# pzou01/unitree-rl-gym

Measured on AMD Instinct MI355X. Metric: env-steps/sec + PPO-iter wall-time, Go2 4096 envs/GPU at 1/2/4/8 MI355X, higher is better.
Workload: dtype fp32 env step; bf16 MFMA policy GEMMs (fp32 accumulate); 1 GPU; Go2 flat terrain, 4096 envs/GPU, MLP actor-critic 512-256-128, PPO 24 steps x 5 epochs x 4 mini-batches; num_envs_per_gpu=4096, decimation=4, parallelism=dp1

## Files before the change

### unitree-rl-gym_amd/csrc/ppo_mlp.hip

```cpp
#include <hip/hip_runtime.h>

#include <algorithm>
#include <cstdint>
#include <cstdlib>
#include <type_traits>
#include <string>

#include "../../include/ppo_mlp.h"
#include "pmlp_noise.h"

typedef __bf16 bf16;
typedef bf16 bf16x8 __attribute__((ext_vector_type(8)));
typedef bf16 bf16x4 __attribute__((ext_vector_type(4)));
typedef short shortx4 __attribute__((ext_vector_type(4)));
typedef short shortx8 __attribute__((ext_vector_type(8)));
typedef __attribute__((address_space(3))) shortx4 lds_shortx4;
typedef float floatx16 __attribute__((ext_vector_type(16)));

static thread_local std::string g_err;
static int fail(int code, const std::string& m) {
    g_err = m;
    return code;
}
#define PMLP_CHECK_LAUNCH(what)                                                                       \
// ... 1463 lines not shown
#pragma unroll 8
    for (int i = threadIdx.x; i < nparts; i += PMLP_OPT_THREADS) s += partial[i];
    return block_sum(s, sh);
}
__device__ __forceinline__ size_t frag_index(int r, int c, int ld) {
    return ((((size_t)(r >> 5) * (ld >> 4) + (c >> 4)) * 64 + (r & 31) + 32 * ((c >> 3) & 1)) << 3) + (c & 7);
}
__global__ __launch_bounds__(PMLP_OPT_THREADS) void k_adam(float* __restrict__ p, const float* __restrict__ g,
                                                           float* __restrict__ m, float* __restrict__ v, int64_t n,
                                                           float scale, const float* __restrict__ partial, int nparts,
                                                           const float* step, const float* lr, float max_norm,
                                                           float b1, float b2, float eps, MirrorJobs mj) {
    __shared__ float sh[4];
    const float s = norm_partials_sum(partial, nparts, sh);
    float coef = scale;
    if (max_norm > 0.f) coef = scale * fminf(max_norm / (sqrtf(s) + 1e-6f), 1.f);
    const float t = step[0];
    const float bc1 = 1.f - powf(b1, t), bc2s = sqrtf(1.f - powf(b2, t));
    const float step_size = lr[0] / bc1;
    for (int64_t i = (int64_t)blockIdx.x * PMLP_OPT_THREADS + threadIdx.x; i < n;
         i += (int64_t)gridDim.x * PMLP_OPT_THREADS) {
        float mi = m[i], vi = v[i];
        const float pi = adam_elem(g[i], mi, vi, p[i], coef, b1, b2, eps, step_size, bc2s);
        m[i] = mi;
        v[i] = vi;
        p[i] = pi;
        for (int j = 0; j < mj.n; ++j) {
            const int64_t o = i - mj.off[j];
            if (o >= 0 && o < (int64_t)mj.rows[j] * mj.cols[j]) {
                const int oi = (int)o, r = oi / mj.cols[j], c = oi - r * mj.cols[j];
                mj.dst[j][(size_t)r * mj.ld[j] + c] = (bf16)pi;
                if (mj.frag[j]) mj.frag[j][frag_index(r, c, mj.ld[j])] = (bf16)pi;
            }
        }
    }
}

template <int VEC>
__global__ __launch_bounds__(PMLP_OPT_THREADS) void k_adam_vec(float* __restrict__ p, const float* __restrict__ g,
                                                               float* __restrict__ m, float* __restrict__ v, int64_t n,
                                                               float scale, const float* __restrict__ partial, int nparts,
                                                               const float* step, const float* lr, float max_norm,
                                                               float b1, float b2, float eps, MirrorJobs mj) {
    typedef float vf __attribute__((ext_vector_type(VEC)));
    typedef bf16 vb __attribute__((ext_vector_type(VEC)));
    __shared__ float sh[4];
    const int64_t ng = n / VEC, i0 = (int64_t)blockIdx.x * PMLP_OPT_THREADS + threadIdx.x;
    const int64_t stride = (int64_t)gridDim.x * PMLP_OPT_THREADS;
    vf G, M, V, P;
    if (i0 < ng) {
        G = ((const vf*)g)[i0];
        M = ((const vf*)m)[i0];
        V = ((const vf*)v)[i0];
        P = ((const vf*)p)[i0];
    }
    const float s = norm_partials_sum(partial, nparts, sh);
    float coef = scale;
    if (max_norm > 0.f) coef = scale * fminf(max_norm / (sqrtf(s) + 1e-6f), 1.f);
    const float t = step[0];
    const float bc1 = 1.f - powf(b1, t), bc2s = sqrtf(1.f - powf(b2, t));
    const float step_size = lr[0] / bc1;
    for (int64_t i = i0; i < ng; i += stride) {
        if (i != i0) {
            G = ((const vf*)g)[i];
            M = ((const vf*)m)[i];
            V = ((const vf*)v)[i];
            P = ((const vf*)p)[i];
        }
        vb B;
#pragma unroll
        for (int e = 0; e < VEC; ++e) {
            float me = M[e], ve = V[e];
            P[e] = adam_elem(G[e], me, ve, P[e], coef, b1, b2, eps, step_size, bc2s);
            M[e] = me;
            V[e] = ve;
            B[e] = (bf16)P[e];
        }
        ((vf*)m)[i] = M;
        ((vf*)v)[i] = V;
        ((vf*)p)[i] = P;
        const int64_t e0 = i * VEC;
        for (int j = 0; j < mj.n; ++j) {
            const int64_t o = e0 - mj.off[j];
            if (o >= 0 && o < (int64_t)mj.rows[j] * mj.cols[j]) {
                const int oi = (int)o, r = oi / mj.cols[j], c = oi - r * mj.cols[j];
                *(vb*)(mj.dst[j] + (size_t)r * mj.ld[j] + c) = B;
                if (mj.frag[j]) *(vb*)(mj.frag[j] + frag_index(r, c, mj.ld[j])) = B;
            }
        }
    }
    if (blockIdx.x == 0 && threadIdx.x < n - ng * VEC) {
        const int64_t i = ng * VEC + threadIdx.x;
        float mi = m[i], vi = v[i];
        p[i] = adam_elem(g[i], mi, vi, p[i], coef, b1, b2, eps, step_size, bc2s);
        m[i] = mi;
        v[i] = vi;
    }
}


#define FMLP_MAX_H0 512
#define FMLP_MAX_H1 256
#define FMLP_MAX_K0 256
#define FMLP_THREADS 512

struct FmlpJob {
    const float* x;
    const int64_t* rows;
    int ldx, kx;
    bf16* xa;
    int ldxa;
    const bf16* W[4];
    const float* b[4];
    int N[4];
    int K0;
    bf16* y[3];
    int ldy[3];
    float* out;
    int ldo;
    const bf16* Wf[4];
};
struct FmlpJobs {
    FmlpJob j[2];
    int njobs;
};

template <int R, bool LAST>
__device__ __forceinline__ void fmlp_layer(const bf16* A, int lda, int K, const bf16* __restrict__ W,
                                           const bf16* __restrict__ Wf,
                                           const float* __restrict__ bias, int N, bf16* D, int ldd,
                                           float* __restrict__ out, int ldo, int r0, int M) {
    constexpr int RT = R / 32, NW = FMLP_THREADS / 64;
    const int lane = threadIdx.x & 63, wid = threadIdx.x >> 6;
    const int nct = (N + 31) >> 5, ks = K >> 4;
    for (int ct = wid; ct < nct; ct += NW) {
        floatx16 acc[RT];
#pragma unroll
        for (int i = 0; i < RT; ++i)
#pragma unroll
            for (int t = 0; t < 16; ++t) acc[i][t] = 0.f;
        const int n = ct * 32 + (lane & 31);
        const bool nv = n < N;
        const bf16* wrow = Wf ? Wf + ((size_t)ct * ks * 64 + lane) * 8 : W + (size_t)(nv ? n : 0) * K + 8 * (lane >> 5);
        const int wstep = Wf ? 512 : 16;
        const bf16* arow = A + (lane & 31) * lda + 8 * (lane >> 5);
        constexpr int FG = 4;
        bf16x8 bq[FG], bn[FG];
        auto loadg = [&](int s0, bf16x8(&b)[FG]) {
#if defined(PMLP_FMLP_STAMPS) && PMLP_FMLP_STAMPS == 2
#pragma unroll
            for (int u = 0; u < FG; ++u)
#pragma unroll
                for (int e = 0; e < 8; ++e) b[u][e] = (bf16)(float)(s0 + u + e + lane);
#else
#pragma unroll
            for (int u = 0; u < FG; ++u) b[u] = *(const bf16x8*)(wrow + min(s0 + u, ks - 1) * wstep);
#endif
        };
        auto step = [&](int s, const bf16x8& b) {
#pragma unroll
            for (int i = 0; i < RT; ++i) {
                const bf16x8 af = *(const bf16x8*)(arow + i * 32 * lda + s * 16);
#if defined(PMLP_FMLP_STAMPS) && PMLP_FMLP_STAMPS == 3
                acc[i][s & 15] += (float)af[0] * (float)b[0];
#else
                acc[i] = __builtin_amdgcn_mfma_f32_32x32x16_bf16(b, af, acc[i], 0, 0, 0);
#endif
            }
        };
        auto group = [&](int s0, const bf16x8(&b)[FG]) {
#pragma unroll
            for (int u = 0; u < FG; ++u) step(s0 + u, b[u]);
        };
        auto tail = [&](int s0, const bf16x8(&b)[FG]) {
#pragma unroll
            for (int u = 0; u < FG; ++u)
                if (s0 + u < ks) step(s0 + u, b[u]);
        };
        float bq4[4][4];
#pragma unroll
        for (int q = 0; q < 4; ++q)
#pragma unroll
            for (int c = 0; c < 4; ++c)
                bq4[q][c] = bias ? bias[min(ct * 32 + 8 * q + 4 * (lane >> 5) + c, N - 1)] : 0.f;
        loadg(0, bq);
        int s0 = 0;
        for (; s0 + 2 * FG <= ks; s0 += 2 * FG) {
            loadg(s0 + FG, bn);
            group(s0, bq);
            loadg(s0 + 2 * FG, bq);
            group(s0 + FG, bn);
        }
        if (s0 < ks) {
            loadg(s0 + FG, bn);
            tail(s0, bq);
            tail(s0 + FG, bn);
        }
        const int rl = lane & 31;
#pragma unroll
        for (int q = 0; q < 4; ++q) {
            const int n0 = ct * 32 + 8 * q + 4 * (lane >> 5);
            if (LAST && n0 >= N) continue;
#pragma unroll
            for (int i = 0; i < RT; ++i) {
                const int r = i * 32 + rl;
                if constexpr (LAST) {
                    if (r0 + r < M) {
#pragma unroll
                        for (int c = 0; c < 4; ++c)
                            if (n0 + c < N) out[(size_t)(r0 + r) * ldo + n0 + c] = acc[i][4 * q + c] + bq4[q][c];
                    }
                } else {
                    bf16x4 v;
#pragma unroll
                    for (int c = 0; c < 4; ++c) v[c] = (bf16)elu(acc[i][4 * q + c] + bq4[q][c]);
                    *(bf16x4*)(D + r * ldd + n0) = v;
                }
            }
        }
    }
}

template <int R>
__device__ __forceinline__ void fmlp_store(const bf16* D, int lds_ld, int N, bf16* y, int ldy, int r0, int M) {
    if (!y) return;
    const int cpr = N >> 3;
    for (int i = threadIdx.x; i < R * cpr; i += FMLP_THREADS) {
        const int r = i / cpr, c = (i - r * cpr) * 8;
        if (r0 + r < M) *(uint4*)(y + (size_t)(r0 + r) * ldy + c) = *(const uint4*)(D + r * lds_ld + c);
    }
}

#ifdef PMLP_FMLP_STAMPS
#define FMLP_NSTAMP 20
__device__ unsigned long long g_fmlp_stamps[4096 * FMLP_NSTAMP];
#define FMLP_STAMP(k)                                                                          \
    do {                                                                                       \
        const unsigned long long t_ = __builtin_amdgcn_s_memtime();                             \
        if (threadIdx.x == 0 && blockIdx.x < 4096) g_fmlp_stamps[blockIdx.x * FMLP_NSTAMP + (k)] = t_; \
    } while (0)
extern "C" int pmlp_diag_fmlp_stamps(unsigned long long* host, int n) {
    return hipMemcpyFromSymbol(host, HIP_SYMBOL(g_fmlp_stamps), sizeof(unsigned long long) * n) == hipSuccess ? 0 : -1;
}
#else
#define FMLP_STAMP(k) ((void)(k))
#endif

struct RollStep {
    const float* stdv;
    const float* obs;
    const float* cobs;
    int O, CO, A;
    float *actions_out, *st_actions, *st_logp, *st_mu, *st_sigma, *st_value, *st_obs, *st_cobs;
    int64_t* draw;
    int parity;
    uint64_t seed;
    const float* rew;
    const uint8_t* dones;
    const uint8_t* time_outs;
    const float* prev_value;
    float* st_rew;
    uint8_t* st_dones;
    float gamma;
    pmlp_env_extras ex;
};

__device__ __forceinline__ bool ex_any(const pmlp_env_extras& x) { return x.acc[x.nsum] > 0.f; }
__device__ __forceinline__ bool ex_row(const pmlp_env_extras& x, bool any, int i, const uint8_t* time_outs) {
    bool to = false;
    if (x.carry && any) {
        const uint8_t b = x.time_out[i];
        x.carry[i] = b;
        to = b != 0;
    } else if (time_outs) {
        to = time_outs[i] != 0;
    }
    if (x.push && x.last_root_vel && !x.pushed[x.pushed[2] & 1u]) {
        x.last_root_vel[6 * (size_t)i] = x.vsim[2 * (size_t)i];
        x.last_root_vel[6 * (size_t)i + 1] = x.vsim[2 * (size_t)i + 1];
    }
    return to;
}
__device__ __forceinline__ void ex_once(const pmlp_env_extras& x, bool any, int t) {
#pragma clang fp contract(off)
    if (x.ep_means && t < x.nsum) {
        float m = x.ep_means[t];
        if (any) m = x.acc[t] / fmaxf(x.acc[x.nsum], 1.f) / x.ep_len_s;
        x.ep_means[t] = m;
        if (x.ep_snapshot) x.ep_snapshot[t] = m;
    }
    if (x.level_sum && x.ep_means && t == x.nsum) {
        float m = x.ep_means[x.nsum];
        if (any) m = (float)*x.level_sum / (float)x.num_envs;
        x.ep_means[x.nsum] = m;
        if (x.ep_snapshot) x.ep_snapshot[x.nsum] = m;
    }
    if (t <= x.nsum) x.acc_next[t] = 0.f;
    if (t == 0) {
        x.pushed[(x.pushed[2] + 1u) & 1u] = 0u;
        if (x.step_counter) *x.step_counter += 1;
    }
}

template <int R>
__device__ void roll_epilogue(const FmlpJob& J, int jj, const RollStep& rs, int r0, int M, float* terms) {
#pragma clang fp contract(off)
    const int tid = threadIdx.x;
    if (jj == 0) {
        const uint32_t draw = (uint32_t)rs.draw[rs.parity];
        const uint2 key = make_uint2((uint32_t)rs.seed, (uint32_t)(rs.seed >> 32));
        for (int q = tid; q < R * 4; q += FMLP_THREADS) {
            const int rl = q >> 2, c = q & 3, k0 = 4 * c, i = r0 + rl;
            if (i >= M || k0 >= rs.A) continue;
            const uint4 r = philox4x32(make_uint4(draw, (uint32_t)i, (uint32_t)c, 0x5050u), key);
            const float rad0 = sqrtf(-2.f * logf(u01(r.x))), rad1 = sqrtf(-2.f * logf(u01(r.z)));
            float z[4];
            sincospif(2.f * u01(r.y), &z[1], &z[0]);
            sincospif(2.f * u01(r.w), &z[3], &z[2]);
            z[0] *= rad0; z[1] *= rad0; z[2] *= rad1; z[3] *= rad1;
#pragma unroll
            for (int u = 0; u < 4; ++u) {
                const int k = k0 + u;
                if (k >= rs.A) break;
                const size_t o = (size_t)i * rs.A + k;
                const float sg = rs.stdv[k], mu = J.out[(size_t)i * J.ldo + k];
                const float act = mu + sg * z[u];
                const float d = act - mu;
                terms[rl * 16 + k] = -(d * d) / (2.f * sg * sg) - logf(sg) - kHalfLog2Pi;
                rs.actions_out[o] = act;
                rs.st_actions[o] = act;
                rs.st_mu[o] = mu;
                rs.st_sigma[o] = sg;
            }
        }
        __syncthreads();
        const bool ex = rs.rew && rs.ex.acc;
        const bool any = ex && ex_any(rs.ex);
        if (tid < R && r0 + tid < M) {
            const int i = r0 + tid;
            float logp = 0.f;
            for (int k = 0; k < rs.A; ++k) logp += terms[tid * 16 + k];
            rs.st_logp[i] = logp;
            if (rs.rew) {
                const bool to = ex ? ex_row(rs.ex, any, i, rs.time_outs) : (rs.time_outs && rs.time_outs[i]);
                float rw = rs.rew[i];
                if (rs.time_outs) rw = rw + rs.gamma * (rs.prev_value[i] * (to ? 1.f : 0.f));
                rs.st_rew[i] = rw;
                rs.st_dones[i] = rs.dones[i] ? 1 : 0;
            }
        }
        if (ex && blockIdx.x == 0) ex_once(rs.ex, any, tid);
        const int nrow = min(R, M - r0);
        for (int q = tid; q < nrow * rs.O; q += FMLP_THREADS)
            rs.st_obs[(size_t)r0 * rs.O + q] = rs.obs[(size_t)r0 * rs.O + q];
        if (blockIdx.x == 0 && tid == 0) rs.draw[rs.parity ^ 1] = (int64_t)draw + 1;
    } else {
        if (tid < R && r0 + tid < M) rs.st_value[r0 + tid] = J.out[(size_t)(r0 + tid) * J.ldo];
        if (rs.st_cobs) {
            const int nrow = min(R, M - r0);
            for (int q = tid; q < nrow * rs.CO; q += FMLP_THREADS)
                rs.st_cobs[(size_t)r0 * rs.CO + q] = rs.cobs[(size_t)r0 * rs.CO + q];
        }
    }
}

template <int R, bool ROLL = false, bool LOSS = false, bool WIDE = false>
__global__ __launch_bounds__(FMLP_THREADS) void k_mlp_fwd(FmlpJobs jobs, int M, RollStep rs, LossArgs la = {},
                                                         LossStepOut lo = {}) {
    constexpr int LD0 = FMLP_MAX_H0 + 8, LD1 = FMLP_MAX_H1 + 8;
    constexpr bool XR = R >= 96 && !WIDE;
    constexpr int LDX = 68;
    __shared__ __attribute__((aligned(16))) bf16 Y0[R * LD0];
    __shared__ __attribute__((aligned(16))) bf16 Y1[R * LD1];
    __shared__ __attribute__((aligned(16))) bf16 X[XR ? R * LDX : 8];
    bf16* const xs = XR ? X : Y1;
    const int ldxs = XR ? LDX : LD1;
    const int r0 = blockIdx.x * R;
    const int jb = gridDim.y > 1 ? blockIdx.y : 0, je = gridDim.y > 1 ? blockIdx.y + 1 : jobs.njobs;
    for (int jj = jb; jj < je; ++jj) {
        const FmlpJob& J = jobs.j[jj];
        const int sb = 9 * (jj - jb);
        FMLP_STAMP(sb + 0);
        const FmlpJob& P = jobs.j[jj > 0 ? jj - 1 : 0];
        const bool same_rows = XR && jj > jb && !J.xa && J.x == P.x && J.rows == P.rows && J.ldx == P.ldx &&
                               J.kx == P.kx && J.K0 == P.K0;
        const int cpr = J.K0 >> 3;
        for (int i = threadIdx.x; i < (same_rows ? 0 : R * cpr); i += FMLP_THREADS) {
            const int r = i / cpr, k = (i - r * cpr) * 8, m = r0 + r;
            bf16x8 t;
#pragma unroll
            for (int u = 0; u < 8; ++u) t[u] = (bf16)0.f;
            if (m < M) {
                const float* src = J.x + (size_t)(J.rows ? J.rows[m] : (int64_t)m) * J.ldx + k;
                if (k + 8 <= J.kx && (J.ldx & 3) == 0) {
                    const float4 x0 = *(const float4*)src, x1 = *(const float4*)(src + 4);
                    t[0] = (bf16)x0.x; t[1] = (bf16)x0.y; t[2] = (bf16)x0.z; t[3] = (bf16)x0.w;
                    t[4] = (bf16)x1.x; t[5] = (bf16)x1.y; t[6] = (bf16)x1.z; t[7] = (bf16)x1.w;
                } else {
#pragma unroll
                    for (int u = 0; u < 8; ++u) t[u] = k + u < J.kx ? (bf16)src[u] : (bf16)0.f;
                }
                if (J.xa) *(bf16x8*)(J.xa + (size_t)m * J.ldxa + k) = t;
            }
            *(bf16x8*)(xs + r * ldxs + k) = t;
        }
        __syncthreads();
        FMLP_STAMP(sb + 1);
        fmlp_layer<R, false>(xs, ldxs, J.K0, J.W[0], J.Wf[0], J.b[0], J.N[0], Y0, LD0, nullptr, 0, r0, M);
        FMLP_STAMP(sb + 2);
        __syncthreads();
        fmlp_store<R>(Y0, LD0, J.N[0], J.y[0], J.ldy[0], r0, M);
        FMLP_STAMP(sb + 3);
        fmlp_layer<R, false>(Y0, LD0, J.N[0], J.W[1], J.Wf[1], J.b[1], J.N[1], Y1, LD1, nullptr, 0, r0, M);
        FMLP_STAMP(sb + 4);
        __syncthreads();
        fmlp_store<R>(Y1, LD1, J.N[1], J.y[1], J.ldy[1], r0, M);
        FMLP_STAMP(sb + 5);
        fmlp_layer<R, false>(Y1, LD1, J.N[1], J.W[2], J.Wf[2], J.b[2], J.N[2], Y0, LD0, nullptr, 0, r0, M);
        FMLP_STAMP(sb + 6);
        __syncthreads();
        fmlp_store<R>(Y0, LD0, J.N[2], J.y[2], J.ldy[2], r0, M);
        FMLP_STAMP(sb + 7);
        fmlp_layer<R, true>(Y0, LD0, J.N[2], J.W[3], J.Wf[3], J.b[3], J.N[3], nullptr, 0, J.out, J.ldo, r0, M);
        __syncthreads();
        FMLP_STAMP(sb + 8);
        if constexpr (ROLL) roll_epilogue<R>(J, jj, rs, r0, M, (float*)Y1);
    }
    if constexpr (LOSS) loss_quad_rows<R / 16>(la, lo, r0, blockIdx.x, (float*)Y1);
}

__global__ __launch_bounds__(PMLP_OPT_THREADS) void k_gae(const float* __restrict__ rew,
                                                          const uint8_t* __restrict__ dones,
                                                          const float* __restrict__ values,
                                                          const float* __restrict__ last_values,
                                                          float* __restrict__ ret, float* __restrict__ adv, int T,
                                                          int N, float gamma, float lam, double* __restrict__ partial) {
#pragma clang fp contract(off)
    __shared__ double shd[2][4];
    const int e = blockIdx.x * PMLP_OPT_THREADS + threadIdx.x;
    double s1 = 0.0, s2 = 0.0;
    if (e < N) {
        float a = 0.f;
        for (int t = T - 1; t >= 0; --t) {
            const size_t i = (size_t)t * N + e;
            const float next = t == T - 1 ? last_values[e] : values[i + N];
            const float nt = 1.f - (dones[i] ? 1.f : 0.f);
            const float delta = (rew[i] + (nt * gamma) * next) - values[i];
            a = delta + ((nt * gamma) * lam) * a;
            const float r = a + values[i];
            ret[i] = r;
            const float ad = r - values[i];
            adv[i] = ad;
            s1 += ad;
            s2 += (double)ad * ad;
        }
    }
#pragma unroll
    for (int off = 32; off > 0; off >>= 1) {
        s1 += __shfl_xor(s1, off);
        s2 += __shfl_xor(s2, off);
    }
    if ((threadIdx.x & 63) == 0) {
        shd[0][threadIdx.x >> 6] = s1;
        shd[1][threadIdx.x >> 6] = s2;
    }
    __syncthreads();
    if (threadIdx.x == 0) {
        partial[2 * blockIdx.x] = (shd[0][0] + shd[0][1]) + (shd[0][2] + shd[0][3]);
        partial[2 * blockIdx.x + 1] = (shd[1][0] + shd[1][1]) + (shd[1][2] + shd[1][3]);
    }
}

__global__ __launch_bounds__(PMLP_OPT_THREADS) void k_adv_norm(float* __restrict__ adv, int64_t n,
                                                               const double* __restrict__ partial, int nparts,
                                                               const double* __restrict__ gstats) {
    __shared__ double sh[3];
    if (threadIdx.x == 0) {
        double a = 0.0, b = 0.0, c = (double)n;
        if (gstats) {
            a = gstats[0]; b = gstats[1]; c = gstats[2];
        } else {
            for (int i = 0; i < nparts; ++i) {
                a += partial[2 * i];
                b += partial[2 * i + 1];
            }
        }
        sh[0] = a;
        sh[1] = b;
        sh[2] = c;
    }
    __syncthreads();
    const double cnt = sh[2];
    const double mean = sh[0] / cnt;
    const double var = (sh[1] - cnt * mean * mean) / (cnt - 1.0);
    const float meanf = (float)mean, den = (float)sqrt(var > 0.0 ? var : 0.0) + 1e-8f;
    for (int64_t i = (int64_t)blockIdx.x * PMLP_OPT_THREADS + threadIdx.x; i < n;
         i += (int64_t)gridDim.x * PMLP_OPT_THREADS)
        adv[i] = (adv[i] - meanf) / den;
}


struct ActArgs {
    const float *mu, *stdv, *value, *obs, *cobs;
    float *actions_out, *st_actions, *st_logp, *st_mu, *st_sigma, *st_value, *st_obs, *st_cobs;
    const int64_t* draw;
    uint64_t seed;
    int N, A, O, CO;
};

__global__ __launch_bounds__(256) void k_act(ActArgs a) {
    const int64_t tid = (int64_t)blockIdx.x * blockDim.x + threadIdx.x, nth = (int64_t)gridDim.x * blockDim.x;
    const uint32_t draw = (uint32_t)*a.draw;
    const uint2 key = make_uint2((uint32_t)a.seed, (uint32_t)(a.seed >> 32));
    for (int64_t i = tid; i < a.N; i += nth) {
        float logp = 0.f;
        for (int k0 = 0; k0 < a.A; k0 += 4) {
            const uint4 r = philox4x32(make_uint4(draw, (uint32_t)i, (uint32_t)(k0 >> 2), 0x5050u), key);
            const float rad0 = sqrtf(-2.f * logf(u01(r.x))), rad1 = sqrtf(-2.f * logf(u01(r.z)));
            float z[4];
            sincospif(2.f * u01(r.y), &z[1], &z[0]);
            sincospif(2.f * u01(r.w), &z[3], &z[2]);
            z[0] *= rad0; z[1] *= rad0; z[2] *= rad1; z[3] *= rad1;
#pragma unroll
            for (int u = 0; u < 4; ++u) {
                const int k = k0 + u;
                if (k >= a.A) break;
                const size_t o = (size_t)i * a.A + k;
                const float sg = a.stdv[k], mu = a.mu[o];
                const float act = mu + sg * z[u];
                const float d = act - mu;
                logp += -(d * d) / (2.f * sg * sg) - logf(sg) - kHalfLog2Pi;
                a.actions_out[o] = act;
                a.st_actions[o] = act;
                a.st_mu[o] = mu;
                a.st_sigma[o] = sg;
            }
        }
        a.st_logp[i] = logp;
        a.st_value[i] = a.value[i];
    }
    const int64_t no = (int64_t)a.N * a.O;
    if ((no & 3) == 0 && (((uintptr_t)a.obs | (uintptr_t)a.st_obs) & 15) == 0) {
        for (int64_t j = tid; j < no / 4; j += nth) ((float4*)a.st_obs)[j] = ((const float4*)a.obs)[j];
    } else {
        for (int64_t j = tid; j < no; j += nth) a.st_obs[j] = a.obs[j];
    }
    if (a.st_cobs) {
        const int64_t nc = (int64_t)a.N * a.CO;
        for (int64_t j = tid; j < nc; j += nth) a.st_cobs[j] = a.cobs[j];
    }
}

__global__ __launch_bounds__(256) void k_act4(ActArgs a) {
    __shared__ float terms[64][16];
    const int64_t nth = (int64_t)gridDim.x * blockDim.x;
    const uint32_t draw = (uint32_t)*a.draw;
    const uint2 key = make_uint2((uint32_t)a.seed, (uint32_t)(a.seed >> 32));
    const int le = threadIdx.x >> 2, c = threadIdx.x & 3, k0 = 4 * c;
    const bool vec = (a.A & 3) == 0 &&
                     ((((uintptr_t)a.mu | (uintptr_t)a.actions_out | (uintptr_t)a.st_actions | (uintptr_t)a.st_mu |
                        (uintptr_t)a.st_sigma) & 15) == 0);
    for (int64_t base = (int64_t)blockIdx.x * blockDim.x; base < (int64_t)a.N * 4; base += nth) {
        const int64_t i = (base + threadIdx.x) >> 2;
        if (i < a.N && k0 < a.A) {
            const size_t o = (size_t)i * a.A + k0;
            float act[4], mu[4], sg[4], tm[4];
#pragma unroll
            for (int u = 0; u < 4; ++u) mu[u] = k0 + u < a.A ? a.mu[o + u] : 0.f;
            act_quad(draw, key, (uint32_t)i, c, a.A, a.stdv, mu, act, sg, tm);
#pragma unroll
            for (int u = 0; u < 4; ++u)
                if (k0 + u < a.A) terms[le][k0 + u] = tm[u];
            if (vec) {
                const float4 av = make_float4(act[0], act[1], act[2], act[3]);
                *(float4*)(a.actions_out + o) = av;
                *(float4*)(a.st_actions + o) = av;
                *(float4*)(a.st_mu + o) = make_float4(mu[0], mu[1], mu[2], mu[3]);
                *(float4*)(a.st_sigma + o) = make_float4(sg[0], sg[1], sg[2], sg[3]);
            } else {
                for (int u = 0; u < 4 && k0 + u < a.A; ++u) {
                    a.actions_out[o + u] = act[u];
                    a.st_actions[o + u] = act[u];
                    a.st_mu[o + u] = mu[u];
                    a.st_sigma[o + u] = sg[u];
                }
            }
        }
        __syncthreads();
        if (c == 0 && i < a.N) {
            float logp = 0.f;
            for (int k = 0; k < a.A; ++k) logp += terms[le][k];
            a.st_logp[i] = logp;
            a.st_value[i] = a.value[i];
        }
        __syncthreads();
    }
    const int64_t tid = (int64_t)blockIdx.x * blockDim.x + threadIdx.x;
    const int64_t no = (int64_t)a.N * a.O;
    if ((no & 3) == 0 && (((uintptr_t)a.obs | (uintptr_t)a.st_obs) & 15) == 0) {
        for (int64_t j = tid; j < no / 4; j += nth) ((float4*)a.st_obs)[j] = ((const float4*)a.obs)[j];
    } else {
        for (int64_t j = tid; j < no; j += nth) a.st_obs[j] = a.obs[j];
    }
    if (a.st_cobs) {
        const int64_t nc = (int64_t)a.N * a.CO;
        for (int64_t j = tid; j < nc; j += nth) a.st_cobs[j] = a.cobs[j];
    }
}

struct MemReset {
    float* s[PMLP_MAX_MEM_STATES];
    int n, H;
};

__global__ __launch_bounds__(256) void k_store_step(const float* __restrict__ rew, const uint8_t* __restrict__ dones,
                                                    const uint8_t* time_outs,
                                                    const float* __restrict__ st_value, float* __restrict__ st_rew,
                                                    uint8_t* __restrict__ st_dones, int N, float gamma,
                                                    int64_t* draw, MemReset mr, pmlp_env_extras ex) {
#pragma clang fp contract(off)
    const int i = blockIdx.x * blockDim.x + threadIdx.x;
    const bool any = ex.acc && ex_any(ex);
    if (ex.acc && blockIdx.x == 0) ex_once(ex, any, threadIdx.x);
    if (i < N) {
        const bool to = ex.acc ? ex_row(ex, any, i, time_outs) : (time_outs && time_outs[i]);
        float r = rew[i];
        if (time_outs) r = r + gamma * (st_value[i] * (to ? 1.f : 0.f));
        st_rew[i] = r;
        const bool d = dones[i] != 0;
        st_dones[i] = d ? 1 : 0;
        if (d)
            for (int k = 0; k < mr.n; ++k) {
                float4* h = (float4*)(mr.s[k] + (size_t)i * mr.H);
                for (int j = 0; j < mr.H / 4; ++j) h[j] = make_float4(0.f, 0.f, 0.f, 0.f);
            }
    }
    if (i == 0 && draw) *draw += 1;
}

static int g_glds = 1;
static int glds_on() {
    return g_glds;
}

template <int BM, int BN>
static bool gl_fits(int epi, int mode, const GemmBatch& gb, int njobs) {
    if (!glds_on() || (mode & 1)) return false;
    const bool tnl = epi == PMLP_EPI_PARTIAL_TN, bkn = tnl || (mode & 2);
    if (glds_on() == 2 && !tnl) return false;
    if (glds_on() == 3 && !tnl && epi != PMLP_EPI_BWD_DX) return false;
    if (epi == PMLP_EPI_PARTIAL) return false;
    if (tnl && (BM % 64 || BM > 128)) return false;
    if (bkn && (BN % 64 || BN > 128)) return false;
    for (int i = 0; i < njobs; ++i) {
        const GemmArgs& g = gb.j[i];
        if (g.K % 64 || (tnl && g.ksplit % 64)) return false;
        if (tnl && (g.M % BM || g.lda < g.M)) return false;
        if (bkn && (g.N % BN || g.ldb < g.N)) return false;
    }
    return true;
}

template <int BM, int BN, int WM, int WN>
static void launch(int epi, int mode, const GemmBatch& gb, int njobs, int maxm, int maxn, int maxk, hipStream_t st) {
    dim3 grid((maxm + BM - 1) / BM, (maxn + BN - 1) / BN, njobs * gb.slabs), block(64 * WM * WN);
    const bool af = (mode & 1) != 0, bkn = (mode & 2) != 0;
    constexpr bool km_a = BM % 64 == 0 && BM <= 128, km_b = BN % 64 == 0 && BN <= 128;
    if (gl_fits<BM, BN>(epi, mode, gb, njobs)) {
        switch (epi) {
        case PMLP_EPI_FWD_HIDDEN: hipLaunchKernelGGL((k_gemm_nt<BM, BN, WM, WN, 0, 4, 0, 1>), grid, block, 0, st, gb); return;
        case PMLP_EPI_FWD_OUT: hipLaunchKernelGGL((k_gemm_nt<BM, BN, WM, WN, 1, 4, 0, 1>), grid, block, 0, st, gb); return;
        case PMLP_EPI_BWD_DX:
            if (!bkn) {
                hipLaunchKernelGGL((k_gemm_nt<BM, BN, WM, WN, 2, 4, 0, 1>), grid, block, 0, st, gb);
                return;
            }
            if constexpr (km_b) {
                hipLaunchKernelGGL((k_gemm_nt<BM, BN, WM, WN, 2, 4, 2, 1>), grid, block, 0, st, gb);
                return;
            }
            break;
        case PMLP_EPI_PARTIAL_TN:
            if constexpr (km_a && km_b) {
                if (glds_on() >= 2) hipLaunchKernelGGL((k_gemm_nt<BM, BN, WM, WN, 4, 4, 0, 2>), grid, block, 0, st, gb);
                else hipLaunchKernelGGL((k_gemm_nt<BM, BN, WM, WN, 4, 4, 0, 1>), grid, block, 0, st, gb);
                return;
            }
            break;
        default: break;
        }
    }
    if (epi == PMLP_EPI_FWD_HIDDEN && maxk <= 48 && maxk > 32) {
        if (af) hipLaunchKernelGGL((k_gemm_nt<BM, BN, WM, WN, 0, 3, 1>), grid, block, 0, st, gb);
        else hipLaunchKernelGGL((k_gemm_nt<BM, BN, WM, WN, 0, 3>), grid, block, 0, st, gb);
        return;
    }
    if (epi == PMLP_EPI_BWD_DX && maxk <= 16) {
        if (bkn) hipLaunchKernelGGL((k_gemm_nt<BM, BN, WM, WN, 2, 1, 2>), grid, block, 0, st, gb);
        else hipLaunchKernelGGL((k_gemm_nt<BM, BN, WM, WN, 2, 1>), grid, block, 0, st, gb);
        return;
    }
    switch (epi) {
    case PMLP_EPI_FWD_HIDDEN:
        if (af) hipLaunchKernelGGL((k_gemm_nt<BM, BN, WM, WN, 0, 4, 1>), grid, block, 0, st, gb);
        else hipLaunchKernelGGL((k_gemm_nt<BM, BN, WM, WN, 0>), grid, block, 0, st, gb);
        break;
    case PMLP_EPI_FWD_OUT:
        if (af) hipLaunchKernelGGL((k_gemm_nt<BM, BN, WM, WN, 1, 4, 1>), grid, block, 0, st, gb);
        else hipLaunchKernelGGL((k_gemm_nt<BM, BN, WM, WN, 1>), grid, block, 0, st, gb);
        break;
    case PMLP_EPI_BWD_DX:
        if (bkn) hipLaunchKernelGGL((k_gemm_nt<BM, BN, WM, WN, 2, 4, 2>), grid, block, 0, st, gb);
        else hipLaunchKernelGGL((k_gemm_nt<BM, BN, WM, WN, 2>), grid, block, 0, st, gb);
        break;
    case PMLP_EPI_PARTIAL: hipLaunchKernelGGL((k_gemm_nt<BM, BN, WM, WN, 3>), grid, block, 0, st, gb); break;
    default: hipLaunchKernelGGL((k_gemm_nt<BM, BN, WM, WN, 4>), grid, block, 0, st, gb); break;
    }
}

static bool al16(const void* p) { return ((uintptr_t)p & 15) == 0; }

extern "C" {

PMLP_API const char* pmlp_last_error(void) { return g_err.c_str(); }

PMLP_API int pmlp_set_gemm_staging(int32_t glds) {
    const int prev = glds_on();
    g_glds = glds < 0 ? 0 : (glds > 3 ? 3 : glds);
    return prev;
// ... 699 lines not shown
```

Baseline: 12.74 million env-steps/s.

## Hoist rollout noise and scalar loads into prologue; fuse obs storage into gather

The Philox/Box-Muller noise generation and per-row reward, done, time-out and prev-value loads move to a prologue that runs before the MLP layers, so their latency can overlap the GEMM work instead of sitting serially after it. The input gather loop also writes the fp32 observations straight into rollout storage when the layout matches, which removes the separate re-read-and-copy of obs and critic obs in the epilogue. In exchange the prologue values stay live in registers across the layers, which may raise register pressure, and the time-out path is split into a pre-read step and a post-write step.

```diff
diff --git a/unitree-rl-gym_amd/csrc/ppo_mlp.hip b/unitree-rl-gym_amd/csrc/ppo_mlp.hip
--- a/unitree-rl-gym_amd/csrc/ppo_mlp.hip
+++ b/unitree-rl-gym_amd/csrc/ppo_mlp.hip
@@ -1789,29 +1789,73 @@
     }
 }
 
+__device__ __forceinline__ float* roll_gather_dst(const FmlpJob& J, int jj, const RollStep& rs) {
+    const float* src = jj == 0 ? rs.obs : rs.cobs;
+    float* dst = jj == 0 ? rs.st_obs : rs.st_cobs;
+    const int w = jj == 0 ? rs.O : rs.CO;
+    return (dst && J.x == src && !J.rows && J.ldx == w && J.kx == w) ? dst : nullptr;
+}
+
+struct RollPre {
+    uint32_t draw;
+    float z[4];
+    bool any;
+    float rew, pv;
+    uint8_t done, to;
+};
 template <int R>
-__device__ void roll_epilogue(const FmlpJob& J, int jj, const RollStep& rs, int r0, int M, float* terms) {
+__device__ __forceinline__ RollPre roll_prologue(const RollStep& rs, int r0, int M) {
+#pragma clang fp contract(off)
+    static_assert(R * 4 <= FMLP_THREADS, "one (row, action quad) per thread");
+    const int tid = threadIdx.x;
+    RollPre p{};
+    p.draw = (uint32_t)rs.draw[rs.parity];
+    const bool ex = rs.rew && rs.ex.acc;
+    p.any = ex && ex_any(rs.ex);
+    if (rs.rew && tid < R && r0 + tid < M) {
+        const int i = r0 + tid;
+        p.rew = rs.rew[i];
+        p.done = rs.dones[i];
+        if (rs.time_outs) p.pv = rs.prev_value[i];
+        if (ex && rs.ex.carry && p.any) p.to = rs.ex.time_out[i];
+        else if (rs.time_outs) p.to = rs.time_outs[i];
+    }
+    const int rl = tid >> 2, c = tid & 3, i = r0 + rl;
+    if (tid < R * 4 && i < M && 4 * c < rs.A) {
+        const uint2 key = make_uint2((uint32_t)rs.seed, (uint32_t)(rs.seed >> 32));
+        const uint4 r = philox4x32(make_uint4(p.draw, (uint32_t)i, (uint32_t)c, 0x5050u), key);
+        const float rad0 = sqrtf(-2.f * logf(u01(r.x))), rad1 = sqrtf(-2.f * logf(u01(r.z)));
+        sincospif(2.f * u01(r.y), &p.z[1], &p.z[0]);
+        sincospif(2.f * u01(r.w), &p.z[3], &p.z[2]);
+        p.z[0] *= rad0; p.z[1] *= rad0; p.z[2] *= rad1; p.z[3] *= rad1;
+    }
+    return p;
+}
+__device__ __forceinline__ bool ex_row_post(const pmlp_env_extras& x, bool any, int i, uint8_t b) {
+    if (x.carry && any) x.carry[i] = b;
+    if (x.push && x.last_root_vel && !x.pushed[x.pushed[2] & 1u]) {
+        x.last_root_vel[6 * (size_t)i] = x.vsim[2 * (size_t)i];
+        x.last_root_vel[6 * (size_t)i + 1] = x.vsim[2 * (size_t)i + 1];
+    }
+    return b != 0;
+}
+
+template <int R>
+__device__ void roll_epilogue(const FmlpJob& J, int jj, const RollStep& rs, int r0, int M, float* terms,
+                              const RollPre& pre, bool stored) {
 #pragma clang fp contract(off)
     const int tid = threadIdx.x;
     if (jj == 0) {
-        const uint32_t draw = (uint32_t)rs.draw[rs.parity];
-        const uint2 key = make_uint2((uint32_t)rs.seed, (uint32_t)(rs.seed >> 32));
-        for (int q = tid; q < R * 4; q += FMLP_THREADS) {
-            const int rl = q >> 2, c = q & 3, k0 = 4 * c, i = r0 + rl;
-            if (i >= M || k0 >= rs.A) continue;
-            const uint4 r = philox4x32(make_uint4(draw, (uint32_t)i, (uint32_t)c, 0x5050u), key);
-            const float rad0 = sqrtf(-2.f * logf(u01(r.x))), rad1 = sqrtf(-2.f * logf(u01(r.z)));
-            float z[4];
-            sincospif(2.f * u01(r.y), &z[1], &z[0]);
-            sincospif(2.f * u01(r.w), &z[3], &z[2]);
-            z[0] *= rad0; z[1] *= rad0; z[2] *= rad1; z[3] *= rad1;
+        const uint32_t draw = pre.draw;
+        const int rl = tid >> 2, c = tid & 3, k0 = 4 * c, ir = r0 + rl;
+        if (tid < R * 4 && ir < M && k0 < rs.A) {
 #pragma unroll
             for (int u = 0; u < 4; ++u) {
                 const int k = k0 + u;
                 if (k >= rs.A) break;
-                const size_t o = (size_t)i * rs.A + k;
-                const float sg = rs.stdv[k], mu = J.out[(size_t)i * J.ldo + k];
-                const float act = mu + sg * z[u];
+                const size_t o = (size_t)ir * rs.A + k;
+                const float sg = rs.stdv[k], mu = J.out[(size_t)ir * J.ldo + k];
+                const float act = mu + sg * pre.z[u];
                 const float d = act - mu;
                 terms[rl * 16 + k] = -(d * d) / (2.f * sg * sg) - logf(sg) - kHalfLog2Pi;
                 rs.actions_out[o] = act;
@@ -1822,28 +1866,30 @@
         }
         __syncthreads();
         const bool ex = rs.rew && rs.ex.acc;
-        const bool any = ex && ex_any(rs.ex);
+        const bool any = pre.any;
         if (tid < R && r0 + tid < M) {
             const int i = r0 + tid;
             float logp = 0.f;
             for (int k = 0; k < rs.A; ++k) logp += terms[tid * 16 + k];
             rs.st_logp[i] = logp;
             if (rs.rew) {
-                const bool to = ex ? ex_row(rs.ex, any, i, rs.time_outs) : (rs.time_outs && rs.time_outs[i]);
-                float rw = rs.rew[i];
-                if (rs.time_outs) rw = rw + rs.gamma * (rs.prev_value[i] * (to ? 1.f : 0.f));
+                const bool to = ex ? ex_row_post(rs.ex, any, i, pre.to) : pre.to != 0;
+                float rw = pre.rew;
+                if (rs.time_outs) rw = rw + rs.gamma * (pre.pv * (to ? 1.f : 0.f));
                 rs.st_rew[i] = rw;
-                rs.st_dones[i] = rs.dones[i] ? 1 : 0;
+                rs.st_dones[i] = pre.done ? 1 : 0;
             }
         }
         if (ex && blockIdx.x == 0) ex_once(rs.ex, any, tid);
-        const int nrow = min(R, M - r0);
-        for (int q = tid; q < nrow * rs.O; q += FMLP_THREADS)
-            rs.st_obs[(size_t)r0 * rs.O + q] = rs.obs[(size_t)r0 * rs.O + q];
+        if (!stored) {
+            const int nrow = min(R, M - r0);
+            for (int q = tid; q < nrow * rs.O; q += FMLP_THREADS)
+                rs.st_obs[(size_t)r0 * rs.O + q] = rs.obs[(size_t)r0 * rs.O + q];
+        }
         if (blockIdx.x == 0 && tid == 0) rs.draw[rs.parity ^ 1] = (int64_t)draw + 1;
     } else {
         if (tid < R && r0 + tid < M) rs.st_value[r0 + tid] = J.out[(size_t)(r0 + tid) * J.ldo];
-        if (rs.st_cobs) {
+        if (rs.st_cobs && !stored) {
             const int nrow = min(R, M - r0);
             for (int q = tid; q < nrow * rs.CO; q += FMLP_THREADS)
                 rs.st_cobs[(size_t)r0 * rs.CO + q] = rs.cobs[(size_t)r0 * rs.CO + q];
@@ -1871,6 +1917,13 @@
         const FmlpJob& P = jobs.j[jj > 0 ? jj - 1 : 0];
         const bool same_rows = XR && jj > jb && !J.xa && J.x == P.x && J.rows == P.rows && J.ldx == P.ldx &&
                                J.kx == P.kx && J.K0 == P.K0;
+        RollPre pre{};
+        float* st = nullptr;
+        if constexpr (ROLL) {
+            if (jj == 0) pre = roll_prologue<R>(rs, r0, M);
+            st = roll_gather_dst(J, jj, rs);
+        }
+        const bool st16 = ROLL && ((uintptr_t)st & 15) == 0;
         const int cpr = J.K0 >> 3;
         for (int i = threadIdx.x; i < (same_rows ? 0 : R * cpr); i += FMLP_THREADS) {
             const int r = i / cpr, k = (i - r * cpr) * 8, m = r0 + r;
@@ -1883,9 +1936,25 @@
                     const float4 x0 = *(const float4*)src, x1 = *(const float4*)(src + 4);
                     t[0] = (bf16)x0.x; t[1] = (bf16)x0.y; t[2] = (bf16)x0.z; t[3] = (bf16)x0.w;
                     t[4] = (bf16)x1.x; t[5] = (bf16)x1.y; t[6] = (bf16)x1.z; t[7] = (bf16)x1.w;
+                    if constexpr (ROLL) {
+                        if (st && st16) {
+                            float* d = st + (size_t)m * J.ldx + k;
+                            *(float4*)d = x0;
+                            *(float4*)(d + 4) = x1;
+                        } else if (st) {
+                            float* d = st + (size_t)m * J.ldx + k;
+                            d[0] = x0.x; d[1] = x0.y; d[2] = x0.z; d[3] = x0.w;
+                            d[4] = x1.x; d[5] = x1.y; d[6] = x1.z; d[7] = x1.w;
+                        }
+                    }
                 } else {
 #pragma unroll
-                    for (int u = 0; u < 8; ++u) t[u] = k + u < J.kx ? (bf16)src[u] : (bf16)0.f;
+                    for (int u = 0; u < 8; ++u) {
+                        const float v = k + u < J.kx ? src[u] : 0.f;
+                        t[u] = (bf16)v;
+                        if constexpr (ROLL)
+                            if (st && k + u < J.kx) st[(size_t)m * J.ldx + k + u] = v;
+                    }
                 }
                 if (J.xa) *(bf16x8*)(J.xa + (size_t)m * J.ldxa + k) = t;
             }
@@ -1911,7 +1980,7 @@
         fmlp_layer<R, true>(Y0, LD0, J.N[2], J.W[3], J.Wf[3], J.b[3], J.N[3], nullptr, 0, J.out, J.ldo, r0, M);
         __syncthreads();
         FMLP_STAMP(sb + 8);
-        if constexpr (ROLL) roll_epilogue<R>(J, jj, rs, r0, M, (float*)Y1);
+        if constexpr (ROLL) roll_epilogue<R>(J, jj, rs, r0, M, (float*)Y1, pre, st != nullptr);
     }
     if constexpr (LOSS) loss_quad_rows<R / 16>(la, lo, r0, blockIdx.x, (float*)Y1);
 }
```

Result: no change. 12.86 million env-steps/s (median of 2 runs) (+1.0%).
